# hulop/SfMLocalization

Measured on AMD Instinct MI355X. Metric: query images localized/sec, higher is better.
Workload: dtype u32 popcount (Hamming); f64 geometry; 1 GPU; BASELINE configs[2]: 10000-image / 20000000-descriptor synthetic map, 2000 feats/query, BoW shortlist of 100 views (exact L2 over the 10000 x 500 .bow matrix) then the whole per-query path: brute-force Hamming 2-NN + Lowe ratio -> >=16 filter -> F-matrix AC-RANSAC (25 rounds) -> 2D-3D set -> P3P AC-RANSAC (4096) -> pose; one step = a batch of 256 queries, 20 in flight per GPU; views=10000, rows=20000000, nq=2000, bow_knn=100, batch=256, in_flight_per_gpu=20, parallelism=1 GPU, whole bank, queries_localised=6400/6400

## Files before the change

### include/sfmloc.h

```cpp
#ifndef SFMLOC_H
#define SFMLOC_H

#include <stddef.h>
#include <stdint.h>

#ifdef __cplusplus
extern "C" {
#endif

#define SFMLOC_ABI_VERSION 2
#define SFMLOC_DESC_BYTES 64
#define SFMLOC_NOMATCH 0xFFFFFFFFu
#define SFMLOC_MAX_QUERY_ROWS 65535u

enum {
  SFMLOC_OK = 0,
  SFMLOC_EINVAL = -1,
  SFMLOC_ENODEV = -2,
  SFMLOC_EHIP = -3,
  SFMLOC_EIO = -4,
  SFMLOC_ECAP = -5,
  SFMLOC_ENOMEM = -6
};

// ... 586 lines not shown

enum { SFMLOC_MERGE_SIMILARITY = 0, SFMLOC_MERGE_AFFINE = 1 };

typedef struct sfmloc_merge_params {
  uint64_t seed;
  int device;
  uint32_t rounds_per_launch;
  int profile;
  int reserved;
} sfmloc_merge_params;

typedef struct sfmloc_merge_result {
  double M[12];
  uint32_t has_model;
  uint32_t round;
  uint32_t count;
  uint32_t n_inliers;
} sfmloc_merge_result;

void sfmloc_merge_default_params(sfmloc_merge_params *p);
int sfmloc_merge_ransac(const double *A, const double *B, uint64_t n, double thres, uint64_t rounds, double svd_ratio,
                        int model, uint32_t stream, const sfmloc_merge_params *params, sfmloc_merge_result *out,
                        uint32_t *inliers, uint32_t cap);
int sfmloc_merge_inliers(const double *A, const double *B, uint64_t n, const double *M , double thres,
                         const sfmloc_merge_params *params, uint32_t *idx, uint32_t cap, uint32_t *n_out);
int sfmloc_merge_median_nn(const double *X, uint64_t n, const sfmloc_merge_params *params, double *median);
int sfmloc_merge_transform(const double *M , double *R, uint64_t nR, double *X, uint64_t nX,
                           const sfmloc_merge_params *params);
double sfmloc_merge_last_ms(void);

typedef struct sfmloc_reduce_result {
  uint64_t n_keep, n_absorbed, n_pairs;
  uint32_t rounds, reserved;
} sfmloc_reduce_result;
int sfmloc_reduce_points(const double *X , uint64_t n, const double *A , double thres,
                         uint32_t knn, const sfmloc_merge_params *params, uint32_t *owner , uint32_t *order ,
                         double *dist , sfmloc_reduce_result *out);
double sfmloc_reduce_last_ms(void);

typedef struct sfmloc_matches sfmloc_matches;

int sfmloc_query_from_view(sfmloc_map *map, uint32_t view_index, sfmloc_query **out);

int sfmloc_match_one_to_one(sfmloc_map *map, sfmloc_query *query, const uint32_t *view_sel, uint32_t n_sel);

int sfmloc_match_pairs(sfmloc_map *map, const uint32_t *pairs, uint32_t n_pairs, sfmloc_matches **out);

int sfmloc_track(sfmloc_map *map, uint32_t max_frame_dist, sfmloc_matches **out);

int sfmloc_geometric_pairs(sfmloc_map *map, const uint32_t *pairs, uint32_t n_pairs, const uint64_t *offsets,
                           const uint32_t *match_i, const uint32_t *match_j, sfmloc_matches **out);

uint32_t sfmloc_matches_pairs(const sfmloc_matches *m);
int sfmloc_matches_pair(const sfmloc_matches *m, uint32_t k, uint32_t *view_i, uint32_t *view_j, uint32_t *n);
int sfmloc_matches_read(const sfmloc_matches *m, uint32_t k, uint32_t *i, uint32_t *j, uint32_t cap);
void sfmloc_matches_destroy(sfmloc_matches *m);

int sfmloc_debug_math(int device, int op, const double *in, int n, int in_stride, double *out, int out_stride);
int sfmloc_debug_resect6(sfmloc_map *map, const double *pt2d, const double *pt3d, uint32_t n, uint32_t width,
                         uint32_t height, sfmloc_pose *out, uint32_t *inlier_idx, uint32_t cap);
void sfmloc_debug_fail_p3p_alloc(int k);
void sfmloc_debug_fail_next_alloc(int k);
int sfmloc_debug_k3_list_counts(int device, uint64_t *out, int reset);
int sfmloc_debug_k5_round_counts(int device, uint64_t *out, int reset);
int sfmloc_debug_context_views(sfmloc_context *ctx, uint32_t *views, uint32_t cap, uint32_t *n);

enum {
  SFMLOC_K_HAMMING = 0,
  SFMLOC_K_COMPACT = 1,
  SFMLOC_K_FMATRIX = 2,
  SFMLOC_K_MATCHSET = 3,
  SFMLOC_K_P3P = 4,
  SFMLOC_K_BOW = 5,
  SFMLOC_K_COUNT = 8
};
typedef struct sfmloc_kernel_stats {
  double total_ms[SFMLOC_K_COUNT];
  uint64_t launches[SFMLOC_K_COUNT];
  uint64_t hamming_pairs;
  uint64_t hamming_alg_bytes;
  uint64_t hamming_lane_ops;
  uint64_t hamming_pairs_finished;
  uint64_t hamming_rows_flagged;
} sfmloc_kernel_stats;
int sfmloc_stats_read(sfmloc_map *map, sfmloc_kernel_stats *out);
int sfmloc_stats_reset(sfmloc_map *map);
int sfmloc_set_profile(sfmloc_map *map, int level);

#ifdef __cplusplus
}
#endif
#endif
```

### sfmlocalization_amd/csrc/capi.hip

```cpp
#include <stdarg.h>
#include <stdlib.h>
#include <string.h>

#include <algorithm>
#include <chrono>
#include <exception>
#include <new>

#include "chain_device.h"
#include "sfmloc_internal.h"

namespace sfmloc {

static thread_local char g_err[512] = "";

void set_error(const char *fmt, ...) {
  va_list ap;
  va_start(ap, fmt);
  vsnprintf(g_err, sizeof(g_err), fmt, ap);
  va_end(ap);
}

namespace {

// ... 137 lines not shown
    if (!on) return;
    if (!c->event_pool.empty()) {
      ev = std::move(c->event_pool.back());
      c->event_pool.pop_back();
    } else if (ev.a.create(kTimingEvent) || ev.b.create(kTimingEvent)) {
      on = false;
      return;
    }
    hipEventRecord(ev.a, c->stream);
  }
  ~EventScope() {
    if (!on) return;
    hipEventRecord(ev.b, c->stream);
    c->pending_events.emplace_back(which, std::move(ev));
  }
};

int drain_events(Ctx *c, double *per_kind_ms = nullptr) {
  for (auto &pe : c->pending_events) {
    float ms = 0.f;
    SFM_HIP(hipEventSynchronize(pe.second.b));
    SFM_HIP(hipEventElapsedTime(&ms, pe.second.a, pe.second.b));
    c->stats.total_ms[pe.first] += ms;
    if (per_kind_ms) per_kind_ms[pe.first] += ms;
    c->stats.launches[pe.first] += 1;
    c->event_pool.push_back(std::move(pe.second));
  }
  c->pending_events.clear();
  return SFMLOC_OK;
}

void free_ctx(Ctx *c) {
  if (!c) return;
  if (c->borrowers > 0) {
    c->zombie = true;
    return;
  }
  if (c->stream.own) hipStreamSynchronize(c->stream.own);
  Ctx *lender = c->lender;
  delete c;
  if (lender && --lender->borrowers == 0 && lender->zombie) free_ctx(lender);
}

struct CtxFree {
  void operator()(Ctx *c) const { free_ctx(c); }
};

int make_ctx(Map *m, Ctx **out, Ctx *share = nullptr, bool merge_only = false) {
  *out = nullptr;
  std::unique_ptr<Ctx, CtxFree> owner(new (std::nothrow) Ctx());
  Ctx *c = owner.get();
  SFM_CHECK(c, SFMLOC_ENOMEM, "out of host memory");
  c->map = m;
  if (share) {
    c->own_stream.borrow(share->stream.own);
    c->lender = share;
    ++share->borrowers;
  } else {
    SFM_RC(c->own_stream.create());
  }
  c->stream.own = c->own_stream;
  const hipStream_t s = c->stream;
  const uint64_t n_pad = (uint64_t)m->n_blocks * kBlockRows;
  uint64_t *acct = &c->hbm_bytes;
  c->merge_only = merge_only;
  const bool full = !merge_only;
  if (full) SFM_RC(dev_alloc(acct, c->d_part, (size_t)n_pad));
  SFM_RC(dev_alloc(acct, c->d_view_sel, (size_t)m->n_views + 1));
  SFM_RC(dev_alloc(acct, c->d_view_widx0, (size_t)m->n_views + 1));
  if (full) SFM_RC(dev_alloc(acct, c->d_block_list, (size_t)m->n_blocks));
  SFM_RC(dev_alloc(acct, c->d_view_count, (size_t)m->n_views + 1));
  if (full) SFM_RC(dev_alloc(acct, c->d_match_i, (size_t)m->n_rows));
  if (full) SFM_RC(dev_alloc(acct, c->d_match_key, (size_t)m->n_rows));
  if (full) SFM_RC(dev_alloc(acct, c->d_flagged, (size_t)n_pad));
  SFM_RC(dev_alloc(acct, c->d_n_flagged, (size_t)1));
  if (full) SFM_RC(dev_alloc(acct, c->d_flagmask, (size_t)m->n_blocks + 1));
  c->rows_chunk_cap = m->n_blocks < 4096 ? (m->n_blocks ? m->n_blocks : 1) : 4096;
  if (full) {
    SFM_RC(dev_alloc(acct, c->d_rows_scratch, (size_t)c->rows_chunk_cap * 8 * 64));
    SFM_RC(dev_alloc(acct, c->d_rows_arrivals, (size_t)c->rows_chunk_cap));
    SFM_RC(dev_alloc(acct, c->d_flagged_desc, (size_t)c->rows_chunk_cap * 4 * 64));
    SFM_RC(c->d_rows_arrivals.zero(s));
  }
  SFM_RC(dev_alloc(acct, c->d_k1_counters, (size_t)kSelPairsSlot + 1));
  SFM_RC(c->d_k1_counters.zero(s));
  SFM_RC(dev_alloc(acct, c->d_geo_count, (size_t)m->n_views + 1));
  if (full) SFM_RC(dev_alloc(acct, c->d_geo_idx, (size_t)m->n_rows));
  SFM_RC(dev_alloc(acct, c->d_geo_model, ((size_t)m->n_views + 1) * 10));
  SFM_RC(dev_alloc(acct, c->d_result, sizeof(HostResult)));
  {
    HostResult *r = reinterpret_cast<HostResult *>(c->d_result.get());
    c->d_p3p_state = &r->state;
    c->d_pose = &r->pose;
    c->d_status = &r->status;
    c->d_view_stats = r->view_stats;
    c->d_pair_qfeat = r->pair_qfeat;
    c->d_pair_landmark = r->pair_landmark;
  }
  SFM_RC(dev_alloc(acct, c->d_cand_part, (size_t)kPartHeaderBytes + (size_t)c->cand_cap * sizeof(Candidate)));
  if (full) SFM_RC(dev_alloc(acct, c->d_geo_dist, (size_t)m->n_rows));
  SFM_RC(dev_alloc(acct, c->d_best64, (size_t)65536));
  SFM_RC(dev_alloc(acct, c->d_winner, (size_t)65536));
  SFM_RC(dev_alloc(acct, c->d_ms_n, (size_t)1));
  SFM_RC(dev_alloc(acct, c->d_ms_qfeat, (size_t)65536));
  SFM_RC(dev_alloc(acct, c->d_ms_landmark, (size_t)65536));
  SFM_RC(dev_alloc(acct, c->d_pt2d, (size_t)65536 * 2));
  SFM_RC(dev_alloc(acct, c->d_pt3d, (size_t)65536 * 3));
  SFM_RC(dev_alloc(acct, c->d_hyp_nfa, (size_t)kP3pSlots));
  SFM_RC(dev_alloc(acct, c->d_hyp_err, (size_t)kP3pSlots));
  SFM_RC(dev_alloc(acct, c->d_hyp_model, (size_t)kP3pSlots * 12));
  SFM_RC(dev_alloc(acct, c->d_hyp_k, (size_t)kP3pSlots));
  SFM_RC(dev_alloc(acct, c->d_prep_models, (size_t)kP3pBatchMax * 48));
  SFM_RC(dev_alloc(acct, c->d_prep_nm, (size_t)kP3pBatchMax));
  SFM_RC(ctx_p3p_workspace(c, kP3pMaxN));
  if (m->bow_dim) {
    SFM_RC(dev_alloc(acct, c->d_bow_query, (size_t)m->bow_dim));
    SFM_RC(dev_alloc(acct, c->d_bow_dist, (size_t)m->n_views));
    SFM_RC(dev_alloc(acct, c->d_bow_cand, (size_t)m->n_views));
    SFM_RC(dev_alloc(acct, c->d_bow_sel, (size_t)m->n_views + 1));
  }
  SFM_RC(c->h_pinned.alloc((size_t)2 * m->n_views + m->n_blocks + 16));
  SFM_RC(c->h_result.alloc(1));
  memset(c->h_result, 0, sizeof(HostResult));
  SFM_RC(dev_zero(c->d_status, 1, s));
  SFM_RC(c->d_view_count.zero(s));
  SFM_RC(c->d_geo_count.zero(s));
  SFM_RC(c->d_ms_n.zero(s));
  SFM_RC(c->xev_out.create(kOrderingEvent));
  SFM_RC(c->xev_in.create(kOrderingEvent));
  SFM_RC(dev_zero(c->d_pose, 1, s));
  SFM_RC(dev_zero(c->d_p3p_state, 1, s));
  SFM_RC(dev_zero(c->d_view_stats, 3, s));
  SFM_HIP(hipStreamSynchronize(s));
  *out = owner.release();
  return SFMLOC_OK;
}

void free_map(Map *m) {
  if (!m) return;
  hipSetDevice(m->device);
  for (Ctx *c : m->pool) free_ctx(c);
  free_ctx(m->ctx0);
  delete m;
}


struct QueryResetBody {
  static constexpr int kGangThreads = 256;
  static __device__ __forceinline__ void run(QueryResetArgs R) {
    query_reset_items(R, blockIdx.x * 256 + threadIdx.x, gridDim.x * 256);
  }
};
__global__ __launch_bounds__(256) void k_query_reset(QueryResetArgs R) {
  QueryResetBody::run(R);
}

QueryResetArgs make_reset_args(Ctx *c, const Query *q) {
  QueryResetArgs R;
  R.view_count = c->d_view_count;
  R.geo_count = c->d_geo_count;
  R.n_views = c->map->n_views;
  R.best64 = c->d_best64;
  R.nq = q->n ? q->n : 1;
  R.n_flagged = c->d_n_flagged;
  R.status = c->d_status;
  R.cand_header = reinterpret_cast<uint32_t *>(c->d_cand_part.get());
  R.view_stats = c->d_view_stats;
// ... 1585 lines not shown
  SFM_RC(c->d_ms_landmark.upload(iota.data(), n, cs));
  SFM_RC(c->d_ms_n.upload(&n, 1, cs));
  SFM_HIP(hipStreamSynchronize(cs));
  ctx_set_uncalibrated_camera(c, width, height);
  c->p3p_init_fused = false;
  rc = ctx_resection_begin(c);
  if (!rc) rc = ctx_resection_wait_done(c);
  c->p3p_uncal = false;
  if (rc) return rc;
  const HostResult *h = c->h_result;
  *out = h->pose;
  SFM_CHECK((out->status & 4) == 0, SFMLOC_ECAP, "more than %u 2D-3D correspondences (P3P workspace)", c->p3p_cap);
  if (inlier_idx && out->ok && out->n_inliers > 0) {
    SFM_CHECK(cap >= (uint32_t)out->n_inliers, SFMLOC_ECAP, "sfmloc_debug_resect6: cap %u < %d inliers", cap, out->n_inliers);
    SFM_RC(c->d_inlier_idx.read(inlier_idx, out->n_inliers, cs));
  }
  return SFMLOC_OK;
}

void sfmloc_debug_fail_p3p_alloc(int k) { sfmloc::g_test_fail_alloc.store(k, std::memory_order_relaxed); }
void sfmloc_debug_fail_next_alloc(int k) { sfmloc::g_fail_countdown = k; }

int sfmloc_debug_context_views(sfmloc_context *ctx, uint32_t *views, uint32_t cap, uint32_t *n) {
  SFM_CHECK(ctx && n && (views || cap == 0), SFMLOC_EINVAL, "sfmloc_debug_context_views: bad argument");
  Ctx *c = reinterpret_cast<Ctx *>(ctx);
  SFM_CHECK(!c->stream.gang, SFMLOC_EINVAL, "sfmloc_debug_context_views: the context is recording a gang session");
  SFM_HIP(hipSetDevice(c->map->device));
  const hipStream_t cs = c->stream;
  SFM_HIP(hipStreamSynchronize(cs));
  *n = c->last_n_sel;
  SFM_CHECK(cap >= c->last_n_sel, SFMLOC_ECAP, "sfmloc_debug_context_views: cap %u < %u views", cap, c->last_n_sel);
  if (c->last_all_views) {
    for (uint32_t v = 0; v < c->last_n_sel; ++v) views[v] = v;
  } else if (c->last_n_sel) {
    SFM_RC(c->d_view_sel.read(views, c->last_n_sel, cs));
  }
  return SFMLOC_OK;
}

int sfmloc_debug_math(int device, int op, const double *in, int n, int in_stride, double *out, int out_stride) {
  SFM_CHECK(in && out && n > 0 && in_stride > 0 && out_stride > 0, SFMLOC_EINVAL, "sfmloc_debug_math: bad argument");
  int ndev = 0;
  hipError_t e = hipGetDeviceCount(&ndev);
  SFM_CHECK(e == hipSuccess && ndev > 0, SFMLOC_ENODEV, "no HIP device visible; this library has no CPU fallback");
  SFM_HIP(hipSetDevice(device));
  DevBuf<double> d_in, d_out;
  int rc = d_in.alloc(nullptr, (size_t)n * in_stride);
  if (!rc) rc = d_out.alloc(nullptr, (size_t)n * out_stride);
  if (rc) return rc;
  rc = d_in.upload(in, (size_t)n * in_stride, nullptr);
  if (!rc) rc = d_out.zero(nullptr);
  if (!rc) rc = launch_debug_math(op, d_in, n, in_stride, d_out, out_stride, nullptr);
  if (!rc) rc = d_out.read(out, (size_t)n * out_stride, nullptr);
  return rc;
}

int sfmloc_sync(sfmloc_map *map) {
  SFM_CHECK(map, SFMLOC_EINVAL, "sfmloc_sync: null map");
  Map *m = reinterpret_cast<Map *>(map);
  SFM_HIP(hipSetDevice(m->device));
  SFM_HIP(hipStreamSynchronize(m->ctx0->stream));
  for (Ctx *c : m->pool) SFM_HIP(hipStreamSynchronize(c->stream));
  return SFMLOC_OK;
}

int sfmloc_stats_read(sfmloc_map *map, sfmloc_kernel_stats *out) {
  SFM_CHECK(map && out, SFMLOC_EINVAL, "sfmloc_stats_read: null argument");
  Map *m = reinterpret_cast<Map *>(map);
  SFM_HIP(hipSetDevice(m->device));
  memset(out, 0, sizeof(*out));
  std::vector<Ctx *> all = m->pool;
  all.push_back(m->ctx0);
  for (Ctx *c : all) {
    const hipStream_t cs = c->stream;
    SFM_HIP(hipStreamSynchronize(cs));
    int rc = drain_events(c);
    if (rc) return rc;
    for (int k = 0; k < SFMLOC_K_COUNT; ++k) {
      out->total_ms[k] += c->stats.total_ms[k];
      out->launches[k] += c->stats.launches[k];
    }
    out->hamming_pairs += c->stats.hamming_pairs;
    out->hamming_alg_bytes += c->stats.hamming_alg_bytes;
    unsigned long long k1s[kSelPairsSlot + 1], k1c[2] = {0, 0};
    SFM_RC(c->d_k1_counters.read(k1s, kSelPairsSlot + 1, cs));
    for (int q = 0; q < kK1CounterSlots; ++q) {
      k1c[0] += k1s[2 * q];
      k1c[1] += k1s[2 * q + 1];
    }
    out->hamming_lane_ops += c->stats.hamming_lane_ops + 64ull * k1c[0] * (uint64_t)c->k1_finish_ops;
    out->hamming_pairs_finished += 64ull * k1c[0];
    out->hamming_rows_flagged += k1c[1];
    out->hamming_pairs += k1s[kSelPairsSlot];
  }
  return SFMLOC_OK;
}

int sfmloc_set_profile(sfmloc_map *map, int level) {
  SFM_CHECK(map, SFMLOC_EINVAL, "sfmloc_set_profile: null map");
  SFM_CHECK(level >= 0 && level <= 2, SFMLOC_EINVAL, "sfmloc_set_profile: level %d (0 off, 1 every stage, 2 K1 only)", level);
  reinterpret_cast<Map *>(map)->params.profile = level;
  return SFMLOC_OK;
}

int sfmloc_stats_reset(sfmloc_map *map) {
  SFM_CHECK(map, SFMLOC_EINVAL, "sfmloc_stats_reset: null map");
  Map *m = reinterpret_cast<Map *>(map);
  SFM_HIP(hipSetDevice(m->device));
  std::vector<Ctx *> all = m->pool;
  all.push_back(m->ctx0);
  for (Ctx *c : all) {
    const hipStream_t cs = c->stream;
    SFM_HIP(hipStreamSynchronize(cs));
    int rc = drain_events(c);
    if (rc) return rc;
    memset(&c->stats, 0, sizeof(c->stats));
    SFM_RC(c->d_k1_counters.zero(cs));
  }
  return SFMLOC_OK;
}

}
```

### sfmlocalization_amd/csrc/forms.h

```cpp
#pragma once

#include <math.h>
#include <stdint.h>
#include <stdlib.h>
#include <atomic>

namespace sfmloc {

constexpr int kScreenWaves = 8;
constexpr int kScreenNW = 10;
constexpr uint32_t kScreenHead = 64;
constexpr uint32_t kScreenMinNq = 12 * kScreenHead;
constexpr uint32_t kK1SliceBlocksPerCu = 32;
constexpr uint32_t kK1BatchedBlocksPerCu = 16;

constexpr int kF2MaxM = 512;
constexpr int kF2BigM = 1024;
constexpr int kF2HugeM = 2048;
constexpr int kFMaxM = 2048;
constexpr int kF2Batch = 32;
constexpr int kK3WideViews = 256;
constexpr int kK3WideWaves = 4;

constexpr int kP3pSmallN = 512;
constexpr int kP3pSlots = 512;
constexpr int kP3pFirstBatch = 64;
constexpr int kP3pLaterBatch = 256;
constexpr int kP3pWideBatch = 128;
static_assert(4 * kP3pWideBatch <= kP3pSlots, "a wide round's results are four slots per hypothesis");
constexpr int kP3pLargeBatch = 64;
constexpr int kP3pLaterRounds = 6;
constexpr int kP3pGangRounds = 12;
constexpr int kCreditMax = 64;
constexpr int kP3pSmallAfter = 8;

struct Knobs {
  int k1_qsplit = 0;
  int k1_screen_batch = 0;
  uint32_t k1_screen_head = kScreenHead;
  int k3_wide = 1;
  int k3_wide_2048 = 1;
  int k3_big = 1;
  int k3_wide_waves = kK3WideWaves;
  int k3_waves_alone = 16;
  int k3_waves_shared = 4;
  int p3p_small = 1;
  int p3p_prep_ahead = -1;
  int p3p_adaptive = -1;
  int p3p_adapt_quarters = 12;
  int p3p_adapt_floor = 64;
  int p3p_rounds = 9;
  bool p3p_wide_always = false;
};

inline Knobs read_knobs() {
  const auto env_int = [](const char *name, int dflt) {
    const char *e = getenv(name);
    return e ? atoi(e) : dflt;
  };
  Knobs k;
  k.k1_qsplit = env_int("SFMLOC_K1_QSPLIT", 0);
  k.k1_screen_batch = env_int("SFMLOC_K1_SCREEN_BATCH", 0);
  const int head = env_int("SFMLOC_K1_SCREEN_HEAD", (int)kScreenHead);
  k.k1_screen_head = (head >= 2 && head <= 4 * (int)kScreenHead) ? (uint32_t)head : kScreenHead;
  k.k3_wide = env_int("SFMLOC_K3_WIDE", 1);
  k.k3_wide_2048 = env_int("SFMLOC_K3_WIDE_2048", 1);
  k.k3_big = env_int("SFMLOC_K3_BIG", 1);
  const int wide_waves = env_int("SFMLOC_K3_WIDE_WAVES", kK3WideWaves);
  k.k3_wide_waves = (wide_waves == 4 || wide_waves == 8) ? wide_waves : kK3WideWaves;
  k.k3_waves_alone = env_int("SFMLOC_K3_WAVES_ALONE", 16);
  k.k3_waves_shared = env_int("SFMLOC_K3_WAVES_SHARED", 4);
  k.p3p_small = env_int("SFMLOC_P3P_SMALL", 1);
  k.p3p_prep_ahead = env_int("SFMLOC_P3P_PREP_AHEAD", -1);
  k.p3p_adaptive = env_int("SFMLOC_P3P_ADAPTIVE", -1);
  k.p3p_adapt_quarters = env_int("SFMLOC_P3P_ADAPT_QUARTERS", 12);
  k.p3p_adapt_floor = env_int("SFMLOC_P3P_ADAPT_FLOOR", 64);
  const int rounds = env_int("SFMLOC_P3P_ROUNDS", 9);
  k.p3p_rounds = (rounds >= 1 && rounds <= 64) ? rounds : 9;
  k.p3p_wide_always = env_int("SFMLOC_P3P_WIDE_ALONE", 0) == 2;
  return k;
}
inline const Knobs &knobs() {
  static const Knobs k = read_knobs();
  return k;
}

struct FormCredits {
  std::atomic<int> p3p_wide{0};
  std::atomic<int> p3p_small{0};
  std::atomic<int> k3_huge{0};
  std::atomic<int> k3_big{0};

  static void count_down(std::atomic<int> &c) {
    if (c.load(std::memory_order_relaxed) > 0) c.fetch_sub(1, std::memory_order_relaxed);
  }
  void note_p3p_set(int n) {
    if (n > kP3pSmallN) {
      p3p_wide.store(kCreditMax, std::memory_order_relaxed);
      p3p_small.store(0, std::memory_order_relaxed);
    } else {
      count_down(p3p_wide);
      if (p3p_small.load(std::memory_order_relaxed) < kCreditMax) p3p_small.fetch_add(1, std::memory_order_relaxed);
    }
  }
  void note_k3_largest_view(uint32_t v) {
    if (v > (uint32_t)kF2BigM && v <= (uint32_t)kF2HugeM) k3_huge.store(kCreditMax, std::memory_order_relaxed);
    else count_down(k3_huge);
    if (v > (uint32_t)kF2BigM) k3_big.store(0, std::memory_order_relaxed);
    else if (v > (uint32_t)kF2MaxM) k3_big.store(kCreditMax, std::memory_order_relaxed);
    else count_down(k3_big);
  }
};

struct K1In {
  uint32_t nq = 0, n_work_blocks = 0, split = 1;
  int n_cu = 256;
  bool use_list = false;
  bool exact_rows = false, k1_mfma = true;
  bool may_slice = true;
};
enum class K1Form {
  kExact,
  kLean,
  kBatchedTail,
  kMfma,
  kShortlist,
};
struct K1Plan {
  K1Form form = K1Form::kExact;
  int exact_waves = 0;
  uint32_t slices = 1, head = 0;
  bool shared_head = false;
  bool clear_flagmask = false;
  uint64_t lane_ops_per_row = 0;
  int finish_ops = 0;
  bool screened() const { return form != K1Form::kExact; }
};

inline uint32_t k1_slices(const K1In &in, const Knobs &k) {
  const uint32_t head = k.k1_screen_head;
  uint32_t slices = 1;
  if ((uint64_t)in.n_work_blocks < (uint64_t)kK1SliceBlocksPerCu * (uint64_t)in.n_cu) {
    const uint32_t wg_per_slice = (in.n_work_blocks + kScreenWaves - 1) / kScreenWaves;
    const bool batched = in.n_work_blocks < kK1BatchedBlocksPerCu * (uint32_t)in.n_cu;
    const double places = (double)((batched ? 3 : 4) * in.n_cu);
    double best = 1e30;
    for (uint32_t s = 1; s <= 8; ++s) {
      if (s > 1 && (in.nq <= head || (in.nq - head) / s < 3 * head)) break;
      const double g = (double)wg_per_slice * s / places;
      const double full = floor(g), r = g - full;
      const double cost = (full + (r > 0.0 ? 0.45 + 0.55 * r : 0.0)) / s * (1.0 + 0.012 * s);
      if (cost < best) {
        best = cost;
        slices = s;
      }
    }
  }
  if (!in.may_slice) slices = 1;
  if (k.k1_qsplit >= 1 && k.k1_qsplit <= 16) slices = (uint32_t)k.k1_qsplit;
  return slices;
}

inline K1Plan plan_k1(const K1In &in, const Knobs &k) {
  K1Plan p;
  if (in.split != 1 || in.exact_rows || in.nq < kScreenMinNq) {
    const uint64_t wave_blocks = (uint64_t)in.n_work_blocks * in.split;
    p.exact_waves = wave_blocks >= (uint64_t)in.n_cu * kK1SliceBlocksPerCu ? 8 : 4;
    p.lane_ops_per_row = (uint64_t)in.nq * 35;
    return p;
  }
  p.head = k.k1_screen_head;
  p.slices = k1_slices(in, k);
  p.shared_head = p.clear_flagmask = p.slices > 1;
  const bool batched_tail = k.k1_screen_batch ? k.k1_screen_batch == 4 : in.may_slice;
  if (batched_tail && in.n_work_blocks < kK1BatchedBlocksPerCu * (uint32_t)in.n_cu) p.form = K1Form::kBatchedTail;
  else if (in.use_list && p.slices == 1 && in.k1_mfma) p.form = K1Form::kMfma;
  else if (in.use_list) p.form = K1Form::kShortlist;
  else p.form = K1Form::kLean;
  if (p.form == K1Form::kMfma) {
    const uint64_t nq32 = ((uint64_t)in.nq + 31) & ~31ull, head32 = ((uint64_t)p.head + 31) & ~31ull;
    p.lane_ops_per_row = nq32 * 9 / 4 + (head32 < nq32 ? head32 : nq32) * 2 + 112;
    p.finish_ops = 0;
  } else {
    p.lane_ops_per_row = (uint64_t)p.head * 35 + (uint64_t)(in.nq - p.head) * (2 * kScreenNW + 1);
    p.finish_ops = 2 * (16 - kScreenNW) + 5;
  }
  return p;
}

struct K3In {
  uint32_t n_sel = 0;
  int ransac_round = 0;
  bool gang = false, alone = true;
  bool merge_deferred = false;
  int huge_credit = 0, big_credit = 0;
};
enum class K3Merge { kDone, kFolded, kInFront };
struct K3Plan {
  bool wide = false;
  int wide_b0 = 0;
  int wide_waves = 0;
  int max_m = kF2MaxM;
  K3Merge k2 = K3Merge::kDone;
  int waves = 4;
  bool big = false;
  int big_waves = 0;
  int skip_le = kF2MaxM;
};

inline K3Plan plan_k3(const K3In &in, const Knobs &k) {
  K3Plan p;
  const int n_uniform = in.ransac_round - in.ransac_round / 10;
  p.wide_b0 = n_uniform < kF2Batch ? n_uniform : kF2Batch;
  p.wide = p.wide_b0 >= 2 && in.n_sel <= (uint32_t)kK3WideViews && (k.k3_wide == 2 || (k.k3_wide == 1 && !in.gang));
  const bool huge = p.wide && (k.k3_wide_2048 == 2 || (k.k3_wide_2048 == 1 && in.huge_credit > 0));
  if (in.merge_deferred) p.k2 = huge ? K3Merge::kInFront : K3Merge::kFolded;
  if (p.wide) {
    p.max_m = p.skip_le = huge ? kF2HugeM : kF2BigM;
    p.wide_waves = (!huge && k.k3_wide_waves == 8) ? 8 : 4;
    return p;
  }
  const int waves = in.alone ? k.k3_waves_alone : k.k3_waves_shared;
  p.waves = (waves == 16 || waves == 4) ? waves : 8;
  p.big = k.k3_big == 2 || (k.k3_big == 1 && in.big_credit > 0);
  if (p.big) {
    p.big_waves = in.alone ? 8 : 4;
    p.skip_le = kF2BigM;
  }
  return p;
}

struct K5In {
  uint32_t query_n = 0;
  bool uncal = false;
  bool gang = false, others_busy = false;
  bool small = false;
  int small_credit = 0, wide_credit = 0;
};
struct K5QueryPlan {
  bool small = false;
  int first_rounds = 0, later_rounds = kP3pLaterRounds;
  int adaptive_batch = 0;
  int prep_ahead = 0;
  int adapt_quarters = 0, adapt_floor = 0;
};

inline K5QueryPlan plan_k5_query(const K5In &in, const Knobs &k) {
  K5QueryPlan p;
  p.small = k.p3p_small == 2 ||
            (k.p3p_small == 1 && (in.query_n <= (uint32_t)kP3pSmallN || in.small_credit >= kP3pSmallAfter));
  p.first_rounds = in.gang ? (k.p3p_rounds > kP3pGangRounds ? k.p3p_rounds : kP3pGangRounds) : k.p3p_rounds;
  p.adaptive_batch = k.p3p_adaptive >= 0 ? k.p3p_adaptive : (in.others_busy ? 1 : 0);
  p.prep_ahead = k.p3p_prep_ahead == 2 ||
                 (p.adaptive_batch && (k.p3p_prep_ahead == 1 || (k.p3p_prep_ahead < 0 && in.gang)));
  if (in.uncal) p.prep_ahead = 0;
  p.adapt_quarters = k.p3p_adapt_quarters;
  p.adapt_floor = k.p3p_adapt_floor;
  return p;
}

inline bool k5_small_refuted(int set_n) { return set_n > kP3pSmallN; }
// ... 24 lines not shown
```

### sfmlocalization_amd/csrc/hamming_screen_mfma.body.inc

```
  extern __shared__ uint4 qs[];
  const uint32_t lane = threadIdx.x & 63u;
  const uint32_t wave = threadIdx.x >> 6;
  const uint32_t r = lane & 31u, h = lane >> 5;
  const uint32_t w0 = blockIdx.x * WAVES + wave;
  const uint32_t blk = (w0 < n_work_blocks) ? (block_list ? block_list[w0] : w0) : kNoBlock;
  const bool valid = blk != kNoBlock;
  if (!__syncthreads_or(valid)) return;
  const uint32_t plane_stride = lds_rows + 1;
  const uint32_t plus_one = k1_mfma_plus_one_reg();
  v8i B[2][8];
#pragma unroll
  for (int t = 0; t < 2; ++t)
#pragma unroll
    for (int c = 0; c < 2; ++c) {
      uint4 v = make_uint4(0, 0, 0, 0);
      if (valid) v = bank[((uint64_t)blk * 4 + 2 * h + c) * 64 + 32 * t + r];
      B[t][4 * c + 0] = k1_mfma_operand(v.x, plus_one);
      B[t][4 * c + 1] = k1_mfma_operand(v.y, plus_one);
      B[t][4 * c + 2] = k1_mfma_operand(v.z, plus_one);
      B[t][4 * c + 3] = k1_mfma_operand(v.w, plus_one);
    }
  constexpr float kNoDot = -1024.f;
  float best[2] = {kNoDot, kNoDot};
  float hi1[2] = {kNoDot, kNoDot}, hi2[2] = {kNoDot, kNoDot};
  const uint32_t head_rows = min(nq, (head + 31u) & ~31u);
  for (uint32_t j0 = 0; j0 < nq; j0 += lds_rows) {
    const uint32_t cnt = min(lds_rows, nq - j0);
    const uint32_t cnt_pad = (cnt + 31u) & ~31u;
    __syncthreads();
    for (uint32_t i = threadIdx.x; i < cnt_pad * 4; i += WAVES * 64)
      qs[(i & 3u) * plane_stride + (i >> 2)] = qdesc[(uint64_t)j0 * 4 + i];
    __syncthreads();
    if (!valid) continue;
    for (uint32_t jj = 0; jj < cnt_pad; jj += 32) {
      const uint4 a0 = qs[(2 * h) * plane_stride + jj + r], a1 = qs[(2 * h + 1) * plane_stride + jj + r];
      const uint32_t w[8] = {a0.x, a0.y, a0.z, a0.w, a1.x, a1.y, a1.z, a1.w};
      v16f c0 = {0}, c1 = {0};
#pragma unroll
      for (int s = 0; s < 8; ++s) {
        const v8i A = k1_mfma_operand(w[s], plus_one);
        c0 = k1_mfma_step(A, B[0][s], c0);
        c1 = k1_mfma_step(A, B[1][s], c1);
      }
      const uint32_t q0 = j0 + jj;
      if (q0 + 32 > nq) {
#pragma unroll
        for (int reg = 0; reg < 16; ++reg)
          if (q0 + (reg & 3) + 8 * (reg >> 2) + 4 * h >= nq) c0[reg] = kNoDot, c1[reg] = kNoDot;
      }
      if (q0 < head_rows) {
#pragma unroll
        for (int reg = 0; reg < 16; ++reg) {
          hi2[0] = __builtin_amdgcn_fmed3f(hi1[0], hi2[0], c0[reg]);
          hi1[0] = fmaxf(hi1[0], c0[reg]);
          hi2[1] = __builtin_amdgcn_fmed3f(hi1[1], hi2[1], c1[reg]);
          hi1[1] = fmaxf(hi1[1], c1[reg]);
        }
      }
#pragma unroll
      for (int reg = 0; reg < 16; reg += 2) {
        best[0] = fmaxf(fmaxf(best[0], c0[reg]), c0[reg + 1]);
        best[1] = fmaxf(fmaxf(best[1], c1[reg]), c1[reg + 1]);
      }
    }
  }
  if (!valid) return;
  bool flag_t[2];
#pragma unroll
  for (int t = 0; t < 2; ++t) {
    const float o1 = __shfl_xor(hi1[t], 32, 64), o2 = __shfl_xor(hi2[t], 32, 64);
    hi2[t] = __builtin_amdgcn_fmed3f(hi1[t], hi2[t], o1);
    hi1[t] = fmaxf(hi1[t], o1);
    hi2[t] = __builtin_amdgcn_fmed3f(hi1[t], hi2[t], o2);
    best[t] = fmaxf(best[t], __shfl_xor(best[t], 32, 64));
    uint32_t T = 0;
    if (hi2[t] > -600.f) T = (uint32_t)ratio_cnt[k1_mfma_distance_of_dot((int)hi2[t])];
    flag_t[t] = (uint32_t)k1_mfma_distance_of_dot((int)best[t]) < T;
  }
  const unsigned long long mask =
      (__ballot(flag_t[0]) & 0xFFFFFFFFull) | ((unsigned long long)(__ballot(flag_t[1]) & 0xFFFFFFFFull) << 32);
  const bool flag = (mask >> lane) & 1ull;
  const uint32_t pidx = w0 * 64 + lane;
  if (lane == 0) {
    flagmask[w0] = mask;
    if (mask) atomicAdd(&counters[2u * (w0 & (uint32_t)(kK1CounterSlots - 1)) + 1], (unsigned long long)__popcll(mask));
  }
  if (mask) {
    uint32_t base = 0;
    if (lane == 0) base = atomicAdd(n_flagged, (uint32_t)__popcll(mask));
    base = __shfl(base, 0, 64);
    if (flag) {
      const uint32_t slot = base + (uint32_t)__popcll(mask & ((1ull << lane) - 1ull));
      flagged[slot] = make_uint2(pidx, blk * 64 + lane);
      if (slot < flagged_desc_cap) {
#pragma unroll
        for (int c = 0; c < 4; ++c)
          flagged_desc[((uint64_t)(slot >> 6) * 4 + c) * 64 + (slot & 63u)] = bank[((uint64_t)blk * 4 + c) * 64 + lane];
      }
    }
  }
```

### sfmlocalization_amd/csrc/k1_mfma_expand.h

```cpp
#pragma once

#include <stdint.h>

#if defined(__HIPCC__) || defined(__CUDACC__)
#define K1_MFMA_FN __host__ __device__ __forceinline__
#else
#define K1_MFMA_FN static inline
#endif

namespace sfmloc {

constexpr uint32_t kE2m1PlusOne = 0x2u, kE2m1MinusOne = 0xAu;
constexpr uint32_t kE8m0One = 127u;

constexpr uint32_t kE2m1AllPlusOne = 0x22222222u;

K1_MFMA_FN uint32_t k1_mfma_expand_dword(uint32_t w, int j, uint32_t all_plus_one = kE2m1AllPlusOne) {
  return ((w << (3 - j)) & 0x88888888u) | all_plus_one;
}

K1_MFMA_FN void k1_mfma_expand(uint32_t w, uint32_t out[4], uint32_t all_plus_one = kE2m1AllPlusOne) {
  out[0] = k1_mfma_expand_dword(w, 0, all_plus_one);
  out[1] = k1_mfma_expand_dword(w, 1, all_plus_one);
  out[2] = k1_mfma_expand_dword(w, 2, all_plus_one);
  out[3] = k1_mfma_expand_dword(w, 3, all_plus_one);
}

K1_MFMA_FN int k1_mfma_dword_of_step(int h, int s) { return 8 * h + s; }

K1_MFMA_FN int k1_mfma_distance_of_dot(int dot) { return (512 - dot) / 2; }

}
```

### sfmlocalization_amd/csrc/sfmloc_internal.h

```cpp
#pragma once

#include <hip/hip_runtime.h>
#include <stdint.h>
#include <atomic>
#include <exception>
#include <new>
#include <stdio.h>
#include <stdlib.h>
#include <string>
#include <vector>

#include "../../include/sfmloc.h"
#include "chain_device.h"
#include "devmem.h"
#include "forms.h"
#include "gang.h"

namespace sfmloc {

void set_error(const char *fmt, ...);

inline int env_int(const char *name, int dflt) {
  const char *e = getenv(name);
  return e ? atoi(e) : dflt;
}

inline int hip_code(hipError_t e) {
  return (e == hipErrorNoDevice || e == hipErrorInvalidDevice) ? SFMLOC_ENODEV
         : (e == hipErrorOutOfMemory)                          ? SFMLOC_ENOMEM
                                                               : SFMLOC_EHIP;
}

#define SFM_HIP(call)                                                                          \
  do {                                                                                         \
    hipError_t e_ = (call);                                                                    \
    if (e_ != hipSuccess) {                                                                    \
      ::sfmloc::set_error("%s:%d %s -> %s", __FILE__, __LINE__, #call, hipGetErrorString(e_)); \
      return ::sfmloc::hip_code(e_);                                                           \
    }                                                                                          \
  } while (0)

#define SFM_CHECK(cond, code, ...)     \
  do {                                 \
    if (!(cond)) {                     \
      ::sfmloc::set_error(__VA_ARGS__); \
      return (code);                   \
    }                                  \
  } while (0)

#define SFM_RC(call)        \
  do {                      \
    const int rc_ = (call); \
    if (rc_) return rc_;    \
  } while (0)

template <class Handle, class Opaque, class Fill>
inline int make_handle(const char *name, Opaque **out, Fill &&fill) {
  SFM_CHECK(out, SFMLOC_EINVAL, "%s: null argument", name);
  *out = nullptr;
  Handle *h = new (std::nothrow) Handle();
  SFM_CHECK(h, SFMLOC_ENOMEM, "out of host memory");
  int rc;
  try {
    rc = fill(h);
  } catch (const std::bad_alloc &) {
    set_error("%s: out of host memory", name);
    rc = SFMLOC_ENOMEM;
  } catch (const std::exception &e) {
    set_error("%s: %s", name, e.what());
    rc = SFMLOC_EINVAL;
  }
  if (rc) {
    delete h;
    return rc;
  }
  *out = reinterpret_cast<Opaque *>(h);
  return SFMLOC_OK;
}

template <class Options>
inline Options options_or(const Options *opt, void (*defaults)(Options *)) {
  Options o;
  if (opt) o = *opt;
  else defaults(&o);
  return o;
}

constexpr uint32_t kBlockRows = 64;
constexpr int kK1CounterSlots = 64;
constexpr int kSelPairsSlot = 2 * kK1CounterSlots;
constexpr int kP3pMaxN = 4096;
constexpr int kP3pBatchMax = 512;
constexpr uint32_t kPartHeaderBytes = 16;

using Pose = sfmloc_pose;

struct Candidate {
  uint64_t order;
  uint32_t qfeat;
  uint32_t landmark_id;
  double X[3];
};

struct P3pState {
  int n, iter, n_iter, n_reserve, n_index, identity, n_in, done, rounds, status;
  unsigned arrive;
  int finished;
  int batch_limit;
  int switch_iter;
  int prep_iter, prep_n;
  unsigned first_hit;
  double min_nfa, errmax;
  double model[12];
};

struct HostResult;
struct P3pArgs {
  P3pState *state;
  Pose *result;
  const HostResult *record;
  HostResult *host;
  const uint32_t *ms_n, *ms_qfeat, *ms_landmark;
  const double *pt2d, *pt3d;
  double *xn;
  const double *L10;
  float *logc_n, *logc_k;
  int32_t *vec_index, *best_inl;
  double *hyp_nfa;
  int *hyp_k;
  double *hyp_err, *hyp_model;
  int32_t *hyp_inl;
  double *prep_models;
  int *prep_nm;
  int prep_ahead;
  uint32_t *pair_qfeat, *pair_landmark, *inlier_idx;
  uint64_t *ws_key;
  uint32_t *ws_idx;
  double *ws_terms;
  double focal, ppx, ppy;
  int max_iteration, min_resection_points, min_inliers, max_n, refine_pose;
  int adaptive_batch;
  int adapt_quarters, adapt_floor;
  uint64_t seed;
  uint32_t stream;
  int uncal;
};

struct HostResult {
  P3pState state;
  Pose pose;
  int status;
  uint32_t view_stats[3];
  uint32_t pair_qfeat[kP3pMaxN];
  uint32_t pair_landmark[kP3pMaxN];
};

template <class T>
inline int dev_upload(uint64_t *acct, DevBuf<T> &p, const T *h, size_t n, hipStream_t s, size_t min_alloc = 0) {
  SFM_RC(p.alloc(acct, n > min_alloc ? n : min_alloc));
  return p.upload(h, n, s);
}

struct CallScope {
  hipStream_t s = nullptr;
  ~CallScope() {
    if (s) hipStreamSynchronize(s);
  }
  static int use_device(int device) {
    int ndev = 0;
    const hipError_t e = hipGetDeviceCount(&ndev);
    SFM_CHECK(e == hipSuccess && ndev > 0, SFMLOC_ENODEV, "no HIP device visible; this library has no CPU fallback");
    SFM_CHECK(device >= 0 && device < ndev, SFMLOC_EINVAL, "device %d out of range (0..%d)", device, ndev - 1);
    SFM_HIP(hipSetDevice(device));
// ... 348 lines not shown
```

Measured before the change: 4526 queries/s.

## Add partial-dot early-exit screening to MFMA Hamming kernel with adaptive probe

```diff
diff --git a/include/sfmloc.h b/include/sfmloc.h
--- a/include/sfmloc.h
+++ b/include/sfmloc.h
@@ -692,6 +692,7 @@
   uint64_t hamming_lane_ops;
   uint64_t hamming_pairs_finished;
   uint64_t hamming_rows_flagged;
+  uint64_t hamming_pairs_continued;
 } sfmloc_kernel_stats;
 int sfmloc_stats_read(sfmloc_map *map, sfmloc_kernel_stats *out);
 int sfmloc_stats_reset(sfmloc_map *map);
diff --git a/sfmlocalization_amd/csrc/capi.hip b/sfmlocalization_amd/csrc/capi.hip
--- a/sfmlocalization_amd/csrc/capi.hip
+++ b/sfmlocalization_amd/csrc/capi.hip
@@ -243,7 +243,7 @@
     SFM_RC(dev_alloc(acct, c->d_flagged_desc, (size_t)c->rows_chunk_cap * 4 * 64));
     SFM_RC(c->d_rows_arrivals.zero(s));
   }
-  SFM_RC(dev_alloc(acct, c->d_k1_counters, (size_t)kSelPairsSlot + 1));
+  SFM_RC(dev_alloc(acct, c->d_k1_counters, (size_t)kK1CounterWords));
   SFM_RC(c->d_k1_counters.zero(s));
   SFM_RC(dev_alloc(acct, c->d_geo_count, (size_t)m->n_views + 1));
   if (full) SFM_RC(dev_alloc(acct, c->d_geo_idx, (size_t)m->n_rows));
@@ -1995,8 +1995,8 @@
     }
     out->hamming_pairs += c->stats.hamming_pairs;
     out->hamming_alg_bytes += c->stats.hamming_alg_bytes;
-    unsigned long long k1s[kSelPairsSlot + 1], k1c[2] = {0, 0};
-    SFM_RC(c->d_k1_counters.read(k1s, kSelPairsSlot + 1, cs));
+    unsigned long long k1s[kK1CounterWords], k1c[2] = {0, 0};
+    SFM_RC(c->d_k1_counters.read(k1s, kK1CounterWords, cs));
     for (int q = 0; q < kK1CounterSlots; ++q) {
       k1c[0] += k1s[2 * q];
       k1c[1] += k1s[2 * q + 1];
@@ -2005,6 +2005,7 @@
     out->hamming_pairs_finished += 64ull * k1c[0];
     out->hamming_rows_flagged += k1c[1];
     out->hamming_pairs += k1s[kSelPairsSlot];
+    out->hamming_pairs_continued += k1s[kK1MfmaContinuedSlot];
   }
   return SFMLOC_OK;
 }
diff --git a/sfmlocalization_amd/csrc/forms.h b/sfmlocalization_amd/csrc/forms.h
--- a/sfmlocalization_amd/csrc/forms.h
+++ b/sfmlocalization_amd/csrc/forms.h
@@ -38,6 +38,7 @@
   int k1_qsplit = 0;
   int k1_screen_batch = 0;
   uint32_t k1_screen_head = kScreenHead;
+  uint32_t k1_mfma_min_nq = kScreenMinNq;
   int k3_wide = 1;
   int k3_wide_2048 = 1;
   int k3_big = 1;
@@ -63,6 +64,8 @@
   k.k1_screen_batch = env_int("SFMLOC_K1_SCREEN_BATCH", 0);
   const int head = env_int("SFMLOC_K1_SCREEN_HEAD", (int)kScreenHead);
   k.k1_screen_head = (head >= 2 && head <= 4 * (int)kScreenHead) ? (uint32_t)head : kScreenHead;
+  const int mfma_min = env_int("SFMLOC_K1_MFMA_MIN_NQ", (int)kScreenMinNq);
+  k.k1_mfma_min_nq = (mfma_min >= 1 && mfma_min <= (int)kScreenMinNq) ? (uint32_t)mfma_min : kScreenMinNq;
   k.k3_wide = env_int("SFMLOC_K3_WIDE", 1);
   k.k3_wide_2048 = env_int("SFMLOC_K3_WIDE_2048", 1);
   k.k3_big = env_int("SFMLOC_K3_BIG", 1);
@@ -163,12 +166,14 @@
 
 inline K1Plan plan_k1(const K1In &in, const Knobs &k) {
   K1Plan p;
-  if (in.split != 1 || in.exact_rows || in.nq < kScreenMinNq) {
+  const auto exact = [&in]() {
+    K1Plan e;
     const uint64_t wave_blocks = (uint64_t)in.n_work_blocks * in.split;
-    p.exact_waves = wave_blocks >= (uint64_t)in.n_cu * kK1SliceBlocksPerCu ? 8 : 4;
-    p.lane_ops_per_row = (uint64_t)in.nq * 35;
-    return p;
-  }
+    e.exact_waves = wave_blocks >= (uint64_t)in.n_cu * kK1SliceBlocksPerCu ? 8 : 4;
+    e.lane_ops_per_row = (uint64_t)in.nq * 35;
+    return e;
+  };
+  if (in.split != 1 || in.exact_rows || in.nq < k.k1_mfma_min_nq) return exact();
   p.head = k.k1_screen_head;
   p.slices = k1_slices(in, k);
   p.shared_head = p.clear_flagmask = p.slices > 1;
@@ -177,6 +182,7 @@
   else if (in.use_list && p.slices == 1 && in.k1_mfma) p.form = K1Form::kMfma;
   else if (in.use_list) p.form = K1Form::kShortlist;
   else p.form = K1Form::kLean;
+  if (in.nq < kScreenMinNq && p.form != K1Form::kMfma) return exact();
   if (p.form == K1Form::kMfma) {
     const uint64_t nq32 = ((uint64_t)in.nq + 31) & ~31ull, head32 = ((uint64_t)p.head + 31) & ~31ull;
     p.lane_ops_per_row = nq32 * 9 / 4 + (head32 < nq32 ? head32 : nq32) * 2 + 112;
diff --git a/sfmlocalization_amd/csrc/hamming_screen_mfma.body.inc b/sfmlocalization_amd/csrc/hamming_screen_mfma.body.inc
--- a/sfmlocalization_amd/csrc/hamming_screen_mfma.body.inc
+++ b/sfmlocalization_amd/csrc/hamming_screen_mfma.body.inc
@@ -1,9 +1,9 @@
   extern __shared__ uint4 qs[];
-  const uint32_t lane = threadIdx.x & 63u;
-  const uint32_t wave = threadIdx.x >> 6;
-  const uint32_t r = lane & 31u, h = lane >> 5;
+  const uint32_t lane_in = threadIdx.x & 63u;
+  const uint32_t wave = __builtin_amdgcn_readfirstlane(threadIdx.x >> 6);
+  const uint32_t r = lane_in & 31u, h = lane_in >> 5;
   const uint32_t w0 = blockIdx.x * WAVES + wave;
-  const uint32_t blk = (w0 < n_work_blocks) ? (block_list ? block_list[w0] : w0) : kNoBlock;
+  const uint32_t blk = __builtin_amdgcn_readfirstlane((w0 < n_work_blocks) ? (block_list ? block_list[w0] : w0) : kNoBlock);
   const bool valid = blk != kNoBlock;
   if (!__syncthreads_or(valid)) return;
   const uint32_t plane_stride = lds_rows + 1;
@@ -22,8 +22,13 @@
     }
   constexpr float kNoDot = -1024.f;
   float best[2] = {kNoDot, kNoDot};
-  float hi1[2] = {kNoDot, kNoDot}, hi2[2] = {kNoDot, kNoDot};
   const uint32_t head_rows = min(nq, (head + 31u) & ~31u);
+  constexpr float kSlack = (float)k1_mfma_slack(kK1MfmaScreenSteps);
+  float need[2] = {0.f, 0.f};
+  uint32_t n_continued = 0;
+  __shared__ uint32_t s_probe[2];
+  if (threadIdx.x == 0) s_probe[0] = s_probe[1] = 0;
+  bool screen = false;
   for (uint32_t j0 = 0; j0 < nq; j0 += lds_rows) {
     const uint32_t cnt = min(lds_rows, nq - j0);
     const uint32_t cnt_pad = (cnt + 31u) & ~31u;
@@ -31,24 +36,24 @@
     for (uint32_t i = threadIdx.x; i < cnt_pad * 4; i += WAVES * 64)
       qs[(i & 3u) * plane_stride + (i >> 2)] = qdesc[(uint64_t)j0 * 4 + i];
     __syncthreads();
-    if (!valid) continue;
-    for (uint32_t jj = 0; jj < cnt_pad; jj += 32) {
-      const uint4 a0 = qs[(2 * h) * plane_stride + jj + r], a1 = qs[(2 * h + 1) * plane_stride + jj + r];
-      const uint32_t w[8] = {a0.x, a0.y, a0.z, a0.w, a1.x, a1.y, a1.z, a1.w};
-      v16f c0 = {0}, c1 = {0};
+    uint32_t jj = 0;
+    if (j0 == 0 && valid) {
+      float hi1[2] = {kNoDot, kNoDot}, hi2[2] = {kNoDot, kNoDot};
+      for (; jj < head_rows; jj += 32) {
+        const uint4 a0 = qs[(2 * h) * plane_stride + jj + r], a1 = qs[(2 * h + 1) * plane_stride + jj + r];
+        const uint32_t w[8] = {a0.x, a0.y, a0.z, a0.w, a1.x, a1.y, a1.z, a1.w};
+        v16f c0 = {0}, c1 = {0};
 #pragma unroll
-      for (int s = 0; s < 8; ++s) {
-        const v8i A = k1_mfma_operand(w[s], plus_one);
-        c0 = k1_mfma_step(A, B[0][s], c0);
-        c1 = k1_mfma_step(A, B[1][s], c1);
-      }
-      const uint32_t q0 = j0 + jj;
-      if (q0 + 32 > nq) {
+        for (int s = 0; s < kK1MfmaSteps; ++s) {
+          const v8i A = k1_mfma_operand(w[s], plus_one);
+          c0 = k1_mfma_step(A, B[0][s], c0);
+          c1 = k1_mfma_step(A, B[1][s], c1);
+        }
+        if (jj + 32 > nq) {
 #pragma unroll
-        for (int reg = 0; reg < 16; ++reg)
-          if (q0 + (reg & 3) + 8 * (reg >> 2) + 4 * h >= nq) c0[reg] = kNoDot, c1[reg] = kNoDot;
-      }
-      if (q0 < head_rows) {
+          for (int reg = 0; reg < 16; ++reg)
+            if (jj + (reg & 3) + 8 * (reg >> 2) + 4 * h >= nq) c0[reg] = kNoDot, c1[reg] = kNoDot;
+        }
 #pragma unroll
         for (int reg = 0; reg < 16; ++reg) {
           hi2[0] = __builtin_amdgcn_fmed3f(hi1[0], hi2[0], c0[reg]);
@@ -56,26 +61,111 @@
           hi2[1] = __builtin_amdgcn_fmed3f(hi1[1], hi2[1], c1[reg]);
           hi1[1] = fmaxf(hi1[1], c1[reg]);
         }
+#pragma unroll
+        for (int reg = 0; reg < 16; reg += 2) {
+          best[0] = fmaxf(fmaxf(best[0], c0[reg]), c0[reg + 1]);
+          best[1] = fmaxf(fmaxf(best[1], c1[reg]), c1[reg + 1]);
+        }
       }
 #pragma unroll
-      for (int reg = 0; reg < 16; reg += 2) {
-        best[0] = fmaxf(fmaxf(best[0], c0[reg]), c0[reg + 1]);
-        best[1] = fmaxf(fmaxf(best[1], c1[reg]), c1[reg + 1]);
+      for (int t = 0; t < 2; ++t) {
+        const float o1 = __shfl_xor(hi1[t], 32, 64), o2 = __shfl_xor(hi2[t], 32, 64);
+        hi2[t] = __builtin_amdgcn_fmed3f(hi1[t], hi2[t], o1);
+        hi1[t] = fmaxf(hi1[t], o1);
+        hi2[t] = __builtin_amdgcn_fmed3f(hi1[t], hi2[t], o2);
+        uint32_t T = 0;
+        if (hi2[t] > -600.f) T = (uint32_t)ratio_cnt[k1_mfma_distance_of_dot((int)hi2[t])];
+        need[t] = (float)k1_mfma_need_of_threshold((int)T);
       }
     }
+    bool probing = j0 == 0;
+    uint32_t jj_end = probing ? min(cnt_pad, ((head_rows + 31u) & ~31u) + 32u * kK1MfmaProbeTiles) : (screen ? cnt_pad : 0u);
+    for (;;) {
+      const uint32_t jj_first = jj;
+      if (valid)
+        for (; jj < jj_end; jj += 32) {
+          const uint32_t *qw0 = reinterpret_cast<const uint32_t *>(&qs[(2 * h) * plane_stride + jj + r]);
+          const uint32_t *qw1 = reinterpret_cast<const uint32_t *>(&qs[(2 * h + 1) * plane_stride + jj + r]);
+          const uint32_t q0 = j0 + jj;
+          const bool last = q0 + 32 > nq;
+          v16f c0 = {0}, c1 = {0};
+#pragma unroll
+          for (int s = 0; s < kK1MfmaScreenSteps; ++s) {
+            const v8i A = k1_mfma_operand(s < 4 ? qw0[s] : qw1[s - 4], plus_one);
+            c0 = k1_mfma_step(A, B[0][s], c0);
+            c1 = k1_mfma_step(A, B[1][s], c1);
+          }
+          if (last) {
+#pragma unroll
+            for (int reg = 0; reg < 16; ++reg)
+              if (q0 + (reg & 3) + 8 * (reg >> 2) + 4 * h >= nq) c0[reg] = kNoDot, c1[reg] = kNoDot;
+          }
+          float m0 = fmaxf(c0[0], c0[1]), m1 = fmaxf(c1[0], c1[1]);
+#pragma unroll
+          for (int reg = 2; reg < 16; reg += 2) {
+            m0 = fmaxf(fmaxf(m0, c0[reg]), c0[reg + 1]);
+            m1 = fmaxf(fmaxf(m1, c1[reg]), c1[reg + 1]);
+          }
+          if (!__ballot(m0 + kSlack > need[0] || m1 + kSlack > need[1])) continue;
+          ++n_continued;
+#pragma unroll
+          for (int s = kK1MfmaScreenSteps; s < kK1MfmaSteps; ++s) {
+            const v8i A = k1_mfma_operand(s < 4 ? qw0[s] : qw1[s - 4], plus_one);
+            c0 = k1_mfma_step(A, B[0][s], c0);
+            c1 = k1_mfma_step(A, B[1][s], c1);
+          }
+          if (last) {
+#pragma unroll
+            for (int reg = 0; reg < 16; ++reg)
+              if (q0 + (reg & 3) + 8 * (reg >> 2) + 4 * h >= nq) c0[reg] = kNoDot, c1[reg] = kNoDot;
+          }
+#pragma unroll
+          for (int reg = 0; reg < 16; reg += 2) {
+            best[0] = fmaxf(fmaxf(best[0], c0[reg]), c0[reg + 1]);
+            best[1] = fmaxf(fmaxf(best[1], c1[reg]), c1[reg + 1]);
+          }
+        }
+      if (!probing) break;
+      if (valid && jj > jj_first && __builtin_amdgcn_mbcnt_hi(~0u, __builtin_amdgcn_mbcnt_lo(~0u, 0u)) == 0) {
+        atomicAdd(&s_probe[0], n_continued);
+        atomicAdd(&s_probe[1], (jj - jj_first) >> 5);
+      }
+      __syncthreads();
+      screen = kK1MfmaProbeGoOnMax * s_probe[0] <= s_probe[1];
+      probing = false;
+      jj_end = screen ? cnt_pad : jj;
+    }
+    if (valid && !screen)
+      for (; jj < cnt_pad; jj += 32) {
+        const uint4 a0 = qs[(2 * h) * plane_stride + jj + r], a1 = qs[(2 * h + 1) * plane_stride + jj + r];
+        const uint32_t w[8] = {a0.x, a0.y, a0.z, a0.w, a1.x, a1.y, a1.z, a1.w};
+        v16f c0 = {0}, c1 = {0};
+#pragma unroll
+        for (int s = 0; s < kK1MfmaSteps; ++s) {
+          const v8i A = k1_mfma_operand(w[s], plus_one);
+          c0 = k1_mfma_step(A, B[0][s], c0);
+          c1 = k1_mfma_step(A, B[1][s], c1);
+        }
+        const uint32_t q0 = j0 + jj;
+        if (q0 + 32 > nq) {
+#pragma unroll
+          for (int reg = 0; reg < 16; ++reg)
+            if (q0 + (reg & 3) + 8 * (reg >> 2) + 4 * h >= nq) c0[reg] = kNoDot, c1[reg] = kNoDot;
+        }
+#pragma unroll
+        for (int reg = 0; reg < 16; reg += 2) {
+          best[0] = fmaxf(fmaxf(best[0], c0[reg]), c0[reg + 1]);
+          best[1] = fmaxf(fmaxf(best[1], c1[reg]), c1[reg + 1]);
+        }
+      }
   }
   if (!valid) return;
+  const uint32_t lane = __builtin_amdgcn_mbcnt_hi(~0u, __builtin_amdgcn_mbcnt_lo(~0u, 0u));
   bool flag_t[2];
 #pragma unroll
   for (int t = 0; t < 2; ++t) {
-    const float o1 = __shfl_xor(hi1[t], 32, 64), o2 = __shfl_xor(hi2[t], 32, 64);
-    hi2[t] = __builtin_amdgcn_fmed3f(hi1[t], hi2[t], o1);
-    hi1[t] = fmaxf(hi1[t], o1);
-    hi2[t] = __builtin_amdgcn_fmed3f(hi1[t], hi2[t], o2);
     best[t] = fmaxf(best[t], __shfl_xor(best[t], 32, 64));
-    uint32_t T = 0;
-    if (hi2[t] > -600.f) T = (uint32_t)ratio_cnt[k1_mfma_distance_of_dot((int)hi2[t])];
-    flag_t[t] = (uint32_t)k1_mfma_distance_of_dot((int)best[t]) < T;
+    flag_t[t] = best[t] > need[t];
   }
   const unsigned long long mask =
       (__ballot(flag_t[0]) & 0xFFFFFFFFull) | ((unsigned long long)(__ballot(flag_t[1]) & 0xFFFFFFFFull) << 32);
@@ -83,6 +173,7 @@
   const uint32_t pidx = w0 * 64 + lane;
   if (lane == 0) {
     flagmask[w0] = mask;
+    if (n_continued) atomicAdd(&counters[kK1MfmaContinuedSlot], 2048ull * n_continued);
     if (mask) atomicAdd(&counters[2u * (w0 & (uint32_t)(kK1CounterSlots - 1)) + 1], (unsigned long long)__popcll(mask));
   }
   if (mask) {
diff --git a/sfmlocalization_amd/csrc/k1_mfma_expand.h b/sfmlocalization_amd/csrc/k1_mfma_expand.h
--- a/sfmlocalization_amd/csrc/k1_mfma_expand.h
+++ b/sfmlocalization_amd/csrc/k1_mfma_expand.h
@@ -30,4 +30,15 @@
 
 K1_MFMA_FN int k1_mfma_distance_of_dot(int dot) { return (512 - dot) / 2; }
 
+constexpr int kK1MfmaSteps = 8;
+#ifdef SFMLOC_K1_MFMA_SCREEN_STEPS
+constexpr int kK1MfmaScreenSteps = SFMLOC_K1_MFMA_SCREEN_STEPS;
+#else
+constexpr int kK1MfmaScreenSteps = 6;
+#endif
+static_assert(kK1MfmaScreenSteps >= 1 && kK1MfmaScreenSteps <= kK1MfmaSteps, "screening steps");
+constexpr uint32_t kK1MfmaProbeTiles = 4, kK1MfmaProbeGoOnMax = 8;
+constexpr int k1_mfma_slack(int steps) { return 64 * (kK1MfmaSteps - steps); }
+constexpr int k1_mfma_need_of_threshold(int T) { return 512 - 2 * T; }
+
 }
diff --git a/sfmlocalization_amd/csrc/sfmloc_internal.h b/sfmlocalization_amd/csrc/sfmloc_internal.h
--- a/sfmlocalization_amd/csrc/sfmloc_internal.h
+++ b/sfmlocalization_amd/csrc/sfmloc_internal.h
@@ -89,6 +89,8 @@
 constexpr uint32_t kBlockRows = 64;
 constexpr int kK1CounterSlots = 64;
 constexpr int kSelPairsSlot = 2 * kK1CounterSlots;
+constexpr int kK1MfmaContinuedSlot = kSelPairsSlot + 1;
+constexpr int kK1CounterWords = kK1MfmaContinuedSlot + 1;
 constexpr int kP3pMaxN = 4096;
 constexpr int kP3pBatchMax = 512;
 constexpr uint32_t kPartHeaderBytes = 16;
```

Result: faster. 4656 queries/s, median of 6 (+2.9%).
